# AllenInstitute/distributed-vae

Hardware: AMD Instinct MI355X
Metric: cells/sec per train step (fwd+loss+bwd+opt) (higher is better)
Workload: dtype f32; 1 GPU; cpl_mixVAE A=2 arms, synthetic-10x-v1 50000 cells x 5000 genes per GPU, batch 5000/GPU, fp32, H=100 L=10 C=92 S=2, x_drop=0.5, Adam lr=1e-3; global_batch=5000, parallelism=dp1, noise=in-kernel Philox4x32-10

## Files before the change

### distributed-vae_amd/csrc/chain.hip

```cpp
#include "common.hpp"
#include "couple.hpp"
#include <stdlib.h>
#include <type_traits>

namespace mmvae {

constexpr int CH_RT = CHAIN_ROWS / 32;
constexpr int CH_NT = 256 * CH_RT;

struct FwdLayer {
    int64_t w_off, b_off;
    int64_t out_off;
    int K, N, act;
    int64_t obn_mean_off = -1, obn_rstd_off = -1;
    int pl_slot = -1;
};
struct ChainFwdArgs {
    int nlayers;
    FwdLayer L[5];
    int64_t x_off;
    int K0;
    int64_t bn_mean_off, bn_rstd_off;
    int64_t bn_part_off;
    int part_n, part_rows;
    int64_t run_mean_off, run_var_off, run_arm_stride;
    int bn_idx;
    float bn_eps, bn_momentum;
    int64_t stats_part_off;
    int64_t acc_in_off, acc_out_off;
    int64_t planes_off;
    int planes_rows;
    int64_t wpl_off;
    int B, ld, wrows;
    int rows;
    int nblk;
    int64_t per_arm;
};

template <bool VEC>
__device__ __forceinline__ void stage_w_t(float* Ws, int ld, const float* __restrict__ W, int N, int K,
                                          int rows_pad, int cols_pad) {
    const int c4n = cols_pad >> 2;
    const int part = threadIdx.x & 7, r0 = threadIdx.x >> 3;
    for (int cb = 0; cb < c4n; cb += 32) {
        for (int row = r0; row < rows_pad; row += CH_NT / 8) {
            float4 v[4];
#pragma unroll
            for (int j = 0; j < 4; ++j) v[j] = ldg4_t<VEC>(W, K, row, (cb + part + 8 * j) * 4, N, K);
#pragma unroll
            for (int j = 0; j < 4; ++j) {
                const int c = cb + part + 8 * j;
                if (c < c4n) *reinterpret_cast<float4*>(&Ws[row * ld + c * 4]) = v[j];
            }
        }
    }
}
__device__ __forceinline__ void stage_w(float* Ws, int ld, const float* __restrict__ W, int N, int K,
                                        int rows_pad, int cols_pad) {
    const bool vec = (K & 3) == 0 && ((reinterpret_cast<uintptr_t>(W) & 15) == 0);
    if (vec) stage_w_t<true>(Ws, ld, W, N, K, rows_pad, cols_pad);
    else stage_w_t<false>(Ws, ld, W, N, K, rows_pad, cols_pad);
}

constexpr int WQ_N = 4 * (128 / (CH_NT / 8));
__device__ __forceinline__ bool w_split_ok(const float* W, int K, int rows_pad, int cols_pad) {
    return (K & 3) == 0 && ((reinterpret_cast<uintptr_t>(W) & 15) == 0) && rows_pad <= 128 && cols_pad <= 128;
}
__device__ __forceinline__ void w_load(float4 (&wq)[WQ_N], const float* __restrict__ W, int N, int K) {
    const int part = threadIdx.x & 7, r0 = threadIdx.x >> 3;
#pragma unroll
    for (int p = 0; p < WQ_N / 4; ++p)
#pragma unroll
        for (int j = 0; j < 4; ++j) {
            const int row = r0 + (CH_NT / 8) * p, col = (part + 8 * j) * 4;
            const bool ok = row < N && col < K;
            wq[p * 4 + j] = *reinterpret_cast<const float4*>(W + (int64_t)(ok ? row : 0) * K + (ok ? col : 0));
        }
}
__device__ __forceinline__ void w_store(float* Ws, int ld, const float4 (&wq)[WQ_N], int N, int K, int rows_pad, int cols_pad) {
    const int part = threadIdx.x & 7, r0 = threadIdx.x >> 3, c4n = cols_pad >> 2;
#pragma unroll
    for (int p = 0; p < WQ_N / 4; ++p)
#pragma unroll
        for (int j = 0; j < 4; ++j) {
            const int row = r0 + (CH_NT / 8) * p, c = part + 8 * j;
            const bool ok = row < N && c * 4 < K;
            const float4 q = wq[p * 4 + j];
            const float4 v = make_float4(ok ? q.x : 0.f, ok ? q.y : 0.f, ok ? q.z : 0.f, ok ? q.w : 0.f);
            if (c < c4n && row < rows_pad) *reinterpret_cast<float4*>(&Ws[row * ld + c * 4]) = v;
        }
}

typedef __bf16 bf16x8c __attribute__((ext_vector_type(8)));
typedef unsigned u32x4c __attribute__((ext_vector_type(4)));
constexpr int PLS = 128 * 128;
constexpr int WP_N = 3 * ((128 * 16) / CH_NT);
__device__ __forceinline__ void wp_load(u32x4c (&wq)[WP_N], const unsigned short* __restrict__ Wg, int N, int K) {
    const int kc_n = rup(K, 16) >> 3;
#pragma unroll
    for (int pl = 0; pl < 3; ++pl)
#pragma unroll
        for (int i = 0; i < WP_N / 3; ++i) {
            const int idx = threadIdx.x + CH_NT * i, row = idx >> 4, kc = idx & 15;
            const bool ok = row < N && kc < kc_n;
            wq[pl * (WP_N / 3) + i] = *reinterpret_cast<const u32x4c*>(Wg + pl * PLS + (ok ? row : 0) * 128 + (ok ? kc : 0) * 8);
        }
}
__device__ __forceinline__ void wp_store(unsigned* Wp, int wpl, int ldp, const u32x4c (&wq)[WP_N], int N, int K) {
    const int kc_n = rup(K, 16) >> 3;
#pragma unroll
    for (int pl = 0; pl < 3; ++pl)
#pragma unroll
        for (int i = 0; i < WP_N / 3; ++i) {
            const int idx = threadIdx.x + CH_NT * i, row = idx >> 4, kc = idx & 15;
            if (row < N && kc < kc_n) *reinterpret_cast<u32x4c*>(Wp + pl * wpl + row * ldp + kc * 4) = wq[pl * (WP_N / 3) + i];
        }
}
__device__ __forceinline__ void mma_nt_x3(f32x16& acc, const unsigned* Xp, int xpl, const unsigned* Wp, int wpl, int ldp,
                                          int a_row0, int b_row0, int ksteps) {
    const int lane = lane_id();
    const unsigned* pa = Xp + (a_row0 + (lane & 31)) * ldp + 4 * (lane >> 5);
    const unsigned* pb = Wp + (b_row0 + (lane & 31)) * ldp + 4 * (lane >> 5);
    bf16x8c a[3], b[3];
#pragma unroll
    for (int pl = 0; pl < 3; ++pl) {
        a[pl] = __builtin_bit_cast(bf16x8c, *reinterpret_cast<const u32x4c*>(pa + pl * xpl));
        b[pl] = __builtin_bit_cast(bf16x8c, *reinterpret_cast<const u32x4c*>(pb + pl * wpl));
    }
    for (int st = 0; st < ksteps; ++st) {
        const int sn = (st + 1 < ksteps) ? st + 1 : st;
        bf16x8c an[3], bn[3];
#pragma unroll
        for (int pl = 0; pl < 3; ++pl) {
            an[pl] = __builtin_bit_cast(bf16x8c, *reinterpret_cast<const u32x4c*>(pa + pl * xpl + 8 * sn));
            bn[pl] = __builtin_bit_cast(bf16x8c, *reinterpret_cast<const u32x4c*>(pb + pl * wpl + 8 * sn));
        }
        acc = __builtin_amdgcn_mfma_f32_32x32x16_bf16(a[2], b[0], acc, 0, 0, 0);
        acc = __builtin_amdgcn_mfma_f32_32x32x16_bf16(a[0], b[2], acc, 0, 0, 0);
        acc = __builtin_amdgcn_mfma_f32_32x32x16_bf16(a[1], b[1], acc, 0, 0, 0);
        acc = __builtin_amdgcn_mfma_f32_32x32x16_bf16(a[1], b[0], acc, 0, 0, 0);
        acc = __builtin_amdgcn_mfma_f32_32x32x16_bf16(a[0], b[1], acc, 0, 0, 0);
        acc = __builtin_amdgcn_mfma_f32_32x32x16_bf16(a[0], b[0], acc, 0, 0, 0);
#pragma unroll
        for (int pl = 0; pl < 3; ++pl) { a[pl] = an[pl]; b[pl] = bn[pl]; }
    }
}

template <bool X3>
__device__ __forceinline__ void chain_fwd_body(const ChainFwdArgs& a_in, const float* __restrict__ params,
                                               float* __restrict__ ws, float* __restrict__ bn_running,
                                               int64_t* __restrict__ nbt) {
    const ChainFwdArgs a = a_in;
    extern __shared__ __attribute__((aligned(16))) float smem[];
    constexpr int NPL = X3 ? 3 : 1;
    float* Xs = smem;
    float* Ws = smem + NPL * CHAIN_ROWS * a.ld;
    float* mean_s = Ws + NPL * a.wrows * a.ld;
    float* rstd_s = mean_s + 128;
    unsigned* const Xp = reinterpret_cast<unsigned*>(Xs);
    unsigned* const Wp = reinterpret_cast<unsigned*>(Ws);
    const int xpl = CHAIN_ROWS * a.ld, wpl = a.wrows * a.ld;
    const int arm = blockIdx.y, blk = blockIdx.x, b0 = blk * a.rows;
    const int tid = threadIdx.x, lane = tid & 63, wv = tid >> 6, rt = wv >> 2, ct = wv & 3;
    const int B = a.B, ld = a.ld;
    const int nvalid = min(a.rows, B - b0);
    const int Rlim = b0 + nvalid;
    const float* P = params + (int64_t)arm * a.per_arm;

    float4 wq[X3 ? 1 : WQ_N];
    u32x4c wq3[X3 ? WP_N : 1];
    bool wq_valid = false;
    const unsigned short* const WPL = reinterpret_cast<const unsigned short*>(ws + (X3 ? a.wpl_off : 0)) + (int64_t)arm * PL_SMALL_SLOTS * 3 * PLS;
    {
        const FwdLayer L0 = a.L[0];
        if constexpr (X3) {
            wq_valid = true;
            wp_load(wq3, WPL + (int64_t)L0.pl_slot * 3 * PLS, L0.N, L0.K);
        } else {
            wq_valid = w_split_ok(P + L0.w_off, L0.K, rup(L0.N, 32), rup(L0.K, 8));
            if (wq_valid) w_load(wq, P + L0.w_off, L0.N, L0.K);
        }
    }
    const float* X = ws + a.x_off + (int64_t)arm * B * a.K0;
    const int xc4n = rup(a.K0, X3 ? 16 : 8) >> 2;
    const bool x_early = (a.K0 & 3) == 0 && xc4n <= 32;
    float4 xq[4];
    if (x_early) {
#pragma unroll
        for (int j = 0; j < 4; ++j) xq[j] = ldg4_t<true>(X, a.K0, b0 + (tid >> 3), ((tid & 7) + 8 * j) * 4, Rlim, a.K0);
    }
    if (a.bn_mean_off >= 0) {
        const int K0 = a.K0;
        float mean = 0.f, rstd = 0.f;
        if (a.bn_part_off >= 0) {
            float m2 = 0.f;
            if (a.acc_in_off >= 0) {
                if (tid < K0)
                    acc_mean_m2(reinterpret_cast<const long long*>(ws + a.acc_in_off) + (int64_t)arm * ACC_SET_I64, tid, B, mean, m2);
            } else {
                stats_from_partials<CH_NT>(ws + a.bn_part_off + (int64_t)arm * a.part_n * 2 * K0, a.part_n, B, a.part_rows, K0,
                                           Ws, mean, m2);
            }
            rstd = 1.0f / sqrtf(m2 / (float)B + a.bn_eps);
            if (blk == 0 && tid < K0) {
                ws[a.bn_mean_off + (int64_t)arm * K0 + tid] = mean;
                ws[a.bn_rstd_off + (int64_t)arm * K0 + tid] = rstd;
                if (bn_running) {
                    float* rm = bn_running + a.run_mean_off + arm * a.run_arm_stride;
                    float* rv = bn_running + a.run_var_off + arm * a.run_arm_stride;
                    rm[tid] = (1.f - a.bn_momentum) * rm[tid] + a.bn_momentum * mean;
                    rv[tid] = (1.f - a.bn_momentum) * rv[tid] + a.bn_momentum * (m2 / (float)max(B - 1, 1));
                }
                if (nbt && tid == 0) nbt[arm * MMVAE_N_BN + a.bn_idx] += 1;
            }
        } else if (tid < K0) {
            mean = ws[a.bn_mean_off + (int64_t)arm * K0 + tid];
            rstd = ws[a.bn_rstd_off + (int64_t)arm * K0 + tid];
        }
        if (tid < 128) { mean_s[tid] = tid < K0 ? mean : 0.f; rstd_s[tid] = tid < K0 ? rstd : 0.f; }
        lds_barrier();
    }
    {
        const bool bn = a.bn_mean_off >= 0;
        const int c4n = xc4n;
        const bool vec = (a.K0 & 3) == 0;
        const int part = tid & 7, row = tid >> 3;
        auto stage_x = [&](auto tag) __attribute__((always_inline)) {
            constexpr bool V = decltype(tag)::value;
            for (int cb = 0; cb < c4n; cb += 32) {
                float4 v[4];
#pragma unroll
                for (int j = 0; j < 4; ++j) v[j] = (V && x_early) ? xq[j] : ldg4_t<V>(X, a.K0, b0 + row, (cb + part + 8 * j) * 4, Rlim, a.K0);
#pragma unroll
                for (int j = 0; j < 4; ++j) {
                    const int c = cb + part + 8 * j;
                    float4 o = v[j];
                    if (bn) {
                        const bool rok = b0 + row < Rlim;
                        const int cc = min(c, 31) * 4;
                        const float4 m4 = *reinterpret_cast<const float4*>(&mean_s[cc]);
                        const float4 r4 = *reinterpret_cast<const float4*>(&rstd_s[cc]);
                        o.x = rok ? (o.x - m4.x) * r4.x : 0.f;
                        o.y = rok ? (o.y - m4.y) * r4.y : 0.f;
                        o.z = rok ? (o.z - m4.z) * r4.z : 0.f;
                        o.w = rok ? (o.w - m4.w) * r4.w : 0.f;
                    }
                    if constexpr (X3) {
                        if (c < c4n) {
                            unsigned w0[3], w1[3];
                            split3(o.x, o.y, w0);
                            split3(o.z, o.w, w1);
#pragma unroll
                            for (int pl = 0; pl < 3; ++pl)
                                *reinterpret_cast<uint2*>(Xp + pl * xpl + row * ld + c * 2) = make_uint2(w0[pl], w1[pl]);
                        }
                    } else {
                        if (c < c4n) *reinterpret_cast<float4*>(&Xs[row * ld + c * 4]) = o;
                    }
                }
            }
        };
        if (vec) stage_x(VecTag{});
        else stage_x(ScalarTag{});
    }
    for (int l = 0; l < a.nlayers; ++l) {
        const FwdLayer Lr = a.L[l];
        const int K = Lr.K, N = Lr.N, KP = rup(K, 8), NPad = rup(N, 32);
        if constexpr (X3) wp_store(Wp, wpl, ld, wq3, N, K);
        else if (wq_valid) w_store(Ws, ld, wq, N, K, NPad, KP);
        else stage_w(Ws, ld, P + Lr.w_off, N, K, NPad, KP);
        const int col = ct * 32 + (lane & 31);
        const bool active = ct * 32 < NPad;
        const float bias = (active && col < N) ? P[Lr.b_off + col] : 0.f;
        const bool obn = Lr.obn_mean_off >= 0;
        const float omean = (obn && active && col < N) ? ws[Lr.obn_mean_off + (int64_t)arm * N + col] : 0.f;
        const float orstd = (obn && active && col < N) ? ws[Lr.obn_rstd_off + (int64_t)arm * N + col] : 0.f;
        lds_barrier();
        wq_valid = false;
        if (l + 1 < a.nlayers) {
            const FwdLayer Ln = a.L[l + 1];
            if constexpr (X3) {
                wp_load(wq3, WPL + (int64_t)Ln.pl_slot * 3 * PLS, Ln.N, Ln.K);
            } else {
                wq_valid = w_split_ok(P + Ln.w_off, Ln.K, rup(Ln.N, 32), rup(Ln.K, 8));
                if (wq_valid) w_load(wq, P + Ln.w_off, Ln.N, Ln.K);
            }
        }
        f32x16 acc = zero16();
        if constexpr (X3) {
            if (active) mma_nt_x3(acc, Xp, xpl, Wp, wpl, ld, rt * 32, ct * 32, rup(K, 16) >> 4);
        } else {
            if (active) mma_nt(acc, Xs, ld, rt * 32, Ws, ld, ct * 32, KP / 8);
        }
        lds_barrier();
        const bool last = (l + 1 == a.nlayers);
        const bool need_x = !last || a.planes_off >= 0;
        float vals[16];
        if (active) {
            float* out = ws + Lr.out_off + (int64_t)arm * B * N;
#pragma unroll
            for (int r = 0; r < 16; ++r) {
                const int row = rt * 32 + acc_row(r, lane);
                float v = 0.f;
                if (col < N && row < nvalid) {
                    v = acc[r] + bias;
                    if (Lr.act) v = relu_keep_nan(v);
                    out[(int64_t)(b0 + row) * N + col] = v;
                }
                vals[r] = v;
                const float xin = obn ? ((col < N && row < nvalid) ? (v - omean) * orstd : 0.f) : v;
                if constexpr (X3) {
                    const float nbv = __builtin_bit_cast(float, __builtin_amdgcn_update_dpp(0, __builtin_bit_cast(int, xin), 0xF5, 0xF, 0xF, false));
                    if (need_x && !(lane & 1) && col < rup(N, 16)) {
                        unsigned w3[3];
                        split3(xin, nbv, w3);
#pragma unroll
                        for (int pl = 0; pl < 3; ++pl) Xp[pl * xpl + row * ld + (col >> 1)] = w3[pl];
                    }
                } else {
                    if (col < rup(N, 8)) Xs[row * ld + col] = xin;
                }
            }
        }
        if (last && a.stats_part_off >= 0) {
            const int nv = max(0, min(32, nvalid - rt * 32));
            if (active) {
                float s = 0.f;
#pragma unroll
                for (int r = 0; r < 16; ++r) s += vals[r];
                s += __shfl_xor(s, 32, 64);
                const float mean = nv > 0 ? s / (float)nv : 0.f;
                float m2 = 0.f;
#pragma unroll
                for (int r = 0; r < 16; ++r) {
                    const int row = rt * 32 + acc_row(r, lane);
                    if (row < nvalid) { const float dl = vals[r] - mean; m2 += dl * dl; }
                }
                m2 += __shfl_xor(m2, 32, 64);
                if (lane < 32) { Ws[(rt * 2 + 0) * 128 + col] = mean; Ws[(rt * 2 + 1) * 128 + col] = m2; }
            }
            lds_barrier();
            if (rt == 0 && active && lane < 32 && col < N) {
                float n = 0.f, mu = 0.f, M2 = 0.f;
#pragma unroll
                for (int k = 0; k < CH_RT; ++k) {
                    const float nb = (float)max(0, min(32, nvalid - k * 32));
                    if (nb > 0.f) {
                        const float nn = n + nb, dl = Ws[(k * 2 + 0) * 128 + col] - mu;
                        mu += dl * (nb / nn);
                        M2 += Ws[(k * 2 + 1) * 128 + col] + dl * dl * (n * nb / nn);
                        n = nn;
                    }
                }
                if (a.acc_out_off >= 0) {
                    acc_add_stats(reinterpret_cast<long long*>(ws + a.acc_out_off) + (int64_t)arm * ACC_SET_I64, col, n, mu, M2);
                } else {
                    float* p = ws + a.stats_part_off + (((int64_t)arm * a.nblk + blk) * 2) * N;
                    p[col] = mu;
                    p[N + col] = M2;
                }
            }
        }
        lds_barrier();
    }
    if (a.planes_off >= 0) {
        const int N = a.L[a.nlayers - 1].N;
        const int64_t plane = (int64_t)a.planes_rows * 128;
        unsigned short* pl = reinterpret_cast<unsigned short*>(ws + a.planes_off) + (int64_t)arm * 3 * plane;
        const int rows_here = blk == a.nblk - 1 ? a.planes_rows - b0 : a.rows;
        for (int i = tid; i < rows_here * 64; i += CH_NT) {
            const int r = i >> 6, c = (i & 63) * 2;
            unsigned w[3] = {0u, 0u, 0u};
            if constexpr (X3) {
                if (r < nvalid) {
                    if (c < rup(N, 16)) {
#pragma unroll
                        for (int p = 0; p < 3; ++p) w[p] = Xp[p * xpl + r * ld + (c >> 1)];
                    }
                    if (c == N) w[0] |= 0x3F80u;
                    if (c + 1 == N) w[0] |= 0x3F800000u;
                }
            } else {
                float v0 = 0.f, v1 = 0.f;
                if (r < nvalid) {
                    v0 = c < N ? Xs[r * ld + c] : (c == N ? 1.f : 0.f);
                    v1 = c + 1 < N ? Xs[r * ld + c + 1] : (c + 1 == N ? 1.f : 0.f);
                }
                split3(v0, v1, w);
            }
#pragma unroll
            for (int p = 0; p < 3; ++p) *reinterpret_cast<unsigned*>(pl + p * plane + (int64_t)(b0 + r) * 128 + c) = w[p];
        }
    }
}
template <bool X3>
__global__ __launch_bounds__(CH_NT) void k_chain_fwd(const ChainFwdArgs a_in, const float* __restrict__ params,
                                                   float* __restrict__ ws, float* __restrict__ bn_running,
                                                   int64_t* __restrict__ nbt) {
    chain_fwd_body<X3>(a_in, params, ws, bn_running, nbt);
}

struct CoupleRoleArgs {
    int nchain, ncouple;
    int B, C;
    float eps, lam;
    int64_t cc_off, csmp_off, c_mean_off, c_iv_off, couple_part_off, c_acc_off, t_acc_off;
};
template <int AT>
__device__ __forceinline__ void couple_role(const CoupleRoleArgs& cr_in, float* __restrict__ ws) {
    const CoupleRoleArgs cr = cr_in;
    if (2 * (int)blockIdx.x >= cr.ncouple) return;
    extern __shared__ __attribute__((aligned(16))) float smem[];
    const int half = threadIdx.x >> 8, t256 = threadIdx.x & 255;
    constexpr int HALF = 4 * AT * CPL * 64 + AT * CPL * 64 + 8;
    float* sh = smem + half * HALF;
    const int blk = 2 * blockIdx.x + half;
    couple_body<AT>(blk, blk < cr.ncouple, t256, cr.B, cr.C, cr.eps, cr.lam, ws + cr.cc_off, ws + cr.csmp_off, nullptr, 0,
                    reinterpret_cast<const long long*>(ws + cr.c_acc_off), ws + cr.c_mean_off, ws + cr.c_iv_off,
                    ws + cr.couple_part_off, nullptr, reinterpret_cast<long long*>(ws + cr.t_acc_off), sh,
                    sh + 4 * AT * CPL * 64 + AT * CPL * 64, sh + 4 * AT * CPL * 64, nullptr);
}
template <int AT>
__global__ __launch_bounds__(CH_NT) void k_chain_fwd_couple(const ChainFwdArgs a_in, const CoupleRoleArgs cr_in,
                                                          const float* __restrict__ params, float* __restrict__ ws) {
    if ((int)blockIdx.y == AT) {
        couple_role<AT>(cr_in, ws);
        return;
    }
    if ((int)blockIdx.x >= cr_in.nchain) return;
    chain_fwd_body<true>(a_in, params, ws, nullptr, nullptr);
}

struct BwdLayer {
    int64_t w_off;
    int64_t dz_off;
    int64_t act_off;
    int K, N;
    int pl_slot = -1;
};
struct ChainBwdArgs {
    int nlayers;
    BwdLayer L[5];
    int64_t g_off;
    int nslab;
    int64_t slab_stride;
    int64_t bnb_part_off;
    int bnb_n;
    int64_t bn_mean_off, bn_rstd_off;
    int64_t gout_off;
    int64_t part_off;
    int64_t rprev_off, rprev_mean_off, rprev_rstd_off;
    int64_t acc_in_off, acc_out_off, zero_off;
    int zero_n4;
    int64_t wpl_off;
    int B, ld, wrows;
    int64_t per_arm;
};

__device__ __forceinline__ float bn_bwd_val(float g, float av, float mm, float rr, float s1, float s2, float invB) {
#pragma clang fp contract(off)
    const float xh = (av - mm) * rr;
    const float t = g - s1 * invB;
    const float u = xh * (s2 * invB);
    return rr * (t - u);
}
__device__ __forceinline__ float bn_bwd_xhat_acc(float g, float rprev, float mu, float rs, float sum) {
#pragma clang fp contract(off)
    const float xh = (rprev - mu) * rs;
    const float p = g * xh;
    return sum + p;
}

template <bool X3>
__global__ __launch_bounds__(CH_NT) void k_chain_bwd(const ChainBwdArgs a_in, const float* __restrict__ params,
                                                   float* __restrict__ ws) {
    const ChainBwdArgs a = a_in;
    extern __shared__ __attribute__((aligned(16))) float smem[];
    constexpr int NPL = X3 ? 3 : 1;
    float* Gs = smem;
    float* Ws = smem + NPL * CHAIN_ROWS * a.ld;
    float* sums_s = Ws + NPL * a.wrows * a.ld;
    unsigned* const Gp = reinterpret_cast<unsigned*>(Gs);
    unsigned* const Wp = reinterpret_cast<unsigned*>(Ws);
    const int xpl = CHAIN_ROWS * a.ld, wpl = a.wrows * a.ld;
    const int arm = blockIdx.y, blk = blockIdx.x, b0 = blk * CHAIN_ROWS;
    const int tid = threadIdx.x, lane = tid & 63, wv = tid >> 6, rt = wv >> 2, ct = wv & 3;
    const int B = a.B, ld = a.ld;
    const int nvalid = min(CHAIN_ROWS, B - b0);
    const float* P = params + (int64_t)arm * a.per_arm;

    if (a.zero_n4 > 0) grid_zero(ws + a.zero_off, a.zero_n4);
    if (a.bnb_part_off >= 0 && a.acc_in_off >= 0) {
        const int N = a.L[0].N;
        if (tid < 128) {
            double s1 = 0.0, s2 = 0.0;
            if (tid < N) acc_get(reinterpret_cast<const long long*>(ws + a.acc_in_off) + (int64_t)arm * ACC_SET_I64, tid, s1, s2);
            sums_s[tid] = (float)s1;
            sums_s[128 + tid] = (float)s2;
        }
        lds_barrier();
    } else if (a.bnb_part_off >= 0) {
        const int N = a.L[0].N;
        const float r = sums_from_partials<CH_NT>(ws + a.bnb_part_off + (int64_t)arm * a.bnb_n * 2 * N, a.bnb_n, 2 * N,
                                                  reinterpret_cast<double*>(Ws));
        if (tid < 256) sums_s[tid] = 0.f;
        lds_barrier();
        if (tid < 2 * N) sums_s[tid < N ? tid : 128 + tid - N] = r;
        lds_barrier();
    }
    {
        const BwdLayer L0 = a.L[0];
        const int N = L0.N, c4n = rup(N, X3 ? 16 : 8) >> 2;
        const bool has_act = L0.act_off >= 0, bnb = a.bnb_part_off >= 0;
        const float* G = ws + a.g_off + (int64_t)arm * B * N;
        const float* act = has_act ? ws + L0.act_off + (int64_t)arm * B * N : G;
        float* dz = ws + L0.dz_off + (int64_t)arm * B * N;
        const float* mu = bnb ? ws + a.bn_mean_off + (int64_t)arm * N : G;
        const float* rs = bnb ? ws + a.bn_rstd_off + (int64_t)arm * N : G;
        const float invB = 1.f / (float)B;
        const bool vec = (N & 3) == 0;
        const int part = tid & 7, row = tid >> 3;
        const bool rok = row < nvalid;
        auto stage_g = [&](auto tag) __attribute__((always_inline)) {
            constexpr bool V = decltype(tag)::value;
            for (int cb = 0; cb < c4n; cb += 32) {
                float4 gq[4], avq[4], mmq[4], rrq[4];
#pragma unroll
                for (int j = 0; j < 4; ++j) {
                    const int col = (cb + part + 8 * j) * 4;
                    float4 g = make_float4(0.f, 0.f, 0.f, 0.f);
                    auto add_slabs = [&](auto chunk) __attribute__((always_inline)) {
                        constexpr int CHK = decltype(chunk)::value;
                        for (int s0 = 0; s0 < a.nslab; s0 += CHK) {
                            float4 t[CHK];
#pragma unroll
                            for (int sl = 0; sl < CHK; ++sl)
                                t[sl] = ldg4_t<V>(G + (int64_t)min(s0 + sl, a.nslab - 1) * a.slab_stride, N, b0 + row, col, B, N);
#pragma unroll
                            for (int sl = 0; sl < CHK; ++sl) {
                                const bool on = s0 + sl < a.nslab;
                                g.x += on ? t[sl].x : 0.f; g.y += on ? t[sl].y : 0.f; g.z += on ? t[sl].z : 0.f; g.w += on ? t[sl].w : 0.f;
                            }
                        }
                    };
                    if (a.nslab == 1) g = ldg4_t<V>(G, N, b0 + row, col, B, N);
                    else if (a.nslab <= 4) add_slabs(std::integral_constant<int, 4>{});
                    else add_slabs(std::integral_constant<int, 16>{});
                    gq[j] = g;
                    avq[j] = ldg4_t<V>(act, N, b0 + row, col, B, N);
                    mmq[j] = ldg4_t<V>(mu, 0, 0, col, 1, N);
                    rrq[j] = ldg4_t<V>(rs, 0, 0, col, 1, N);
                }
#pragma unroll
                for (int j = 0; j < 4; ++j) {
                    const int c = cb + part + 8 * j, col = c * 4;
                    float4 g = gq[j];
                    const float4 av = avq[j];
                    if (bnb) {
                        const int cs = min(c, 31) * 4;
                        const float4 m1 = *reinterpret_cast<const float4*>(&sums_s[cs]);
                        const float4 m2 = *reinterpret_cast<const float4*>(&sums_s[128 + cs]);
                        const float4 mm = mmq[j], rr = rrq[j];
                        g.x = bn_bwd_val(g.x, av.x, mm.x, rr.x, m1.x, m2.x, invB);
                        g.y = bn_bwd_val(g.y, av.y, mm.y, rr.y, m1.y, m2.y, invB);
                        g.z = bn_bwd_val(g.z, av.z, mm.z, rr.z, m1.z, m2.z, invB);
                        g.w = bn_bwd_val(g.w, av.w, mm.w, rr.w, m1.w, m2.w, invB);
                    }
                    float4 v;
                    v.x = (rok && col < N && (!has_act || av.x > 0.f)) ? g.x : 0.f;
                    v.y = (rok && col + 1 < N && (!has_act || av.y > 0.f)) ? g.y : 0.f;
                    v.z = (rok && col + 2 < N && (!has_act || av.z > 0.f)) ? g.z : 0.f;
                    v.w = (rok && col + 3 < N && (!has_act || av.w > 0.f)) ? g.w : 0.f;
                    if (c < c4n) {
                        if constexpr (X3) {
                            unsigned w0[3], w1[3];
                            split3(v.x, v.y, w0);
                            split3(v.z, v.w, w1);
#pragma unroll
                            for (int pl = 0; pl < 3; ++pl)
                                *reinterpret_cast<uint2*>(Gp + pl * xpl + row * ld + c * 2) = make_uint2(w0[pl], w1[pl]);
                        } else {
                            *reinterpret_cast<float4*>(&Gs[row * ld + col]) = v;
                        }
                        if (rok) {
                            float* o = dz + (int64_t)(b0 + row) * N + col;
                            if (V && col + 3 < N) *reinterpret_cast<float4*>(o) = v;
                            else {
                                if (col < N) o[0] = v.x;
                                if (col + 1 < N) o[1] = v.y;
                                if (col + 2 < N) o[2] = v.z;
                                if (col + 3 < N) o[3] = v.w;
                            }
                        }
                    }
                }
            }
        };
        if (vec) stage_g(VecTag{});
        else stage_g(ScalarTag{});
    }
    float4 wq[X3 ? 1 : WQ_N];
    u32x4c wq3[X3 ? WP_N : 1];
    bool wq_valid = false;
    const unsigned short* const WPL = reinterpret_cast<const unsigned short*>(ws + (X3 ? a.wpl_off : 0)) + (int64_t)arm * PL_SMALL_SLOTS * 3 * PLS;
    if constexpr (X3) wp_load(wq3, WPL + (int64_t)a.L[0].pl_slot * 3 * PLS, a.L[0].K, a.L[0].N);
    for (int l = 0; l < a.nlayers; ++l) {
        const BwdLayer Lr = a.L[l];
        const int K = Lr.K, N = Lr.N, NP8 = rup(N, 8), KPad = rup(K, 32);
        if constexpr (X3) wp_store(Wp, wpl, ld, wq3, K, N);
        else if (wq_valid) w_store(Ws, ld, wq, N, K, NP8, KPad);
        else stage_w(Ws, ld, P + Lr.w_off, N, K, NP8, KPad);
        lds_barrier();
        wq_valid = false;
        if (l + 1 < a.nlayers) {
            const BwdLayer Ln = a.L[l + 1];
            if constexpr (X3) {
                wp_load(wq3, WPL + (int64_t)Ln.pl_slot * 3 * PLS, Ln.K, Ln.N);
            } else {
                wq_valid = w_split_ok(P + Ln.w_off, Ln.K, rup(Ln.N, 8), rup(Ln.K, 32));
                if (wq_valid) w_load(wq, P + Ln.w_off, Ln.N, Ln.K);
            }
        }
        const bool last = (l + 1 == a.nlayers);
        constexpr int NTI = X3 ? 1 : 2;
        float pre[NTI][16];
        {
            const float* src = nullptr;
            if (!last) {
                const BwdLayer Ln = a.L[l + 1];
                src = Ln.act_off >= 0 ? ws + Ln.act_off + (int64_t)arm * B * K : nullptr;
            } else if (a.part_off >= 0) {
                src = ws + a.rprev_off + (int64_t)arm * B * K;
            }
#pragma unroll
            for (int ti = 0; ti < NTI; ++ti) {
                const int col = (ct + 4 * ti) * 32 + (lane & 31);
#pragma unroll
                for (int r = 0; r < 16; ++r) {
                    const int row = rt * 32 + acc_row(r, lane);
                    const bool ok = src && (ct + 4 * ti) * 32 < KPad && col < K && row < nvalid;
                    pre[ti][r] = ok ? src[(int64_t)(b0 + row) * K + col] : (last ? 0.f : 1.f);
                }
            }
        }
        f32x16 accs[NTI];
#pragma unroll
        for (int ti = 0; ti < NTI; ++ti) accs[ti] = zero16();
#pragma unroll
        for (int ti = 0; ti < NTI; ++ti) {
            const int cti = ct + 4 * ti;
            if constexpr (X3) {
                if (cti * 32 < KPad) mma_nt_x3(accs[ti], Gp, xpl, Wp, wpl, ld, rt * 32, cti * 32, rup(N, 16) >> 4);
            } else {
                if (cti * 32 < KPad) mma_nn(accs[ti], Gs, ld, rt * 32, Ws, ld, cti * 32, NP8 / 8);
            }
        }
        lds_barrier();
        float ps1[2] = {0.f, 0.f}, ps2[2] = {0.f, 0.f};
#pragma unroll
        for (int ti = 0; ti < NTI; ++ti) {
            const int cti = ct + 4 * ti;
            if (cti * 32 >= KPad) continue;
            const f32x16 acc = accs[ti];
            const int col = cti * 32 + (lane & 31);
            if (!last) {
                const BwdLayer Ln = a.L[l + 1];
                float* dz = ws + Ln.dz_off + (int64_t)arm * B * K;
#pragma unroll
                for (int r = 0; r < 16; ++r) {
                    const int row = rt * 32 + acc_row(r, lane);
                    const bool ok = col < K && row < nvalid;
                    const float v = (ok && pre[ti][r] > 0.f) ? acc[r] : 0.f;
                    if (ok) dz[(int64_t)(b0 + row) * K + col] = v;
                    if constexpr (X3) {
                        const float nbv = __builtin_bit_cast(float, __builtin_amdgcn_update_dpp(0, __builtin_bit_cast(int, v), 0xF5, 0xF, 0xF, false));
                        if (!(lane & 1) && col < rup(K, 16)) {
                            unsigned w3[3];
                            split3(v, nbv, w3);
#pragma unroll
                            for (int pl = 0; pl < 3; ++pl) Gp[pl * xpl + row * ld + (col >> 1)] = w3[pl];
                        }
                    } else {
                        Gs[row * ld + col] = v;
                    }
                }
            } else {
                float* go = ws + a.gout_off + (int64_t)arm * B * K;
                float s1 = 0.f, s2 = 0.f;
                const bool want = a.part_off >= 0;
                float mu = 0.f, rs = 0.f;
                if (want && col < K) {
                    mu = ws[a.rprev_mean_off + (int64_t)arm * K + col];
                    rs = ws[a.rprev_rstd_off + (int64_t)arm * K + col];
                }
#pragma unroll
                for (int r = 0; r < 16; ++r) {
                    const int row = rt * 32 + acc_row(r, lane);
                    if (col < K && row < nvalid) {
                        go[(int64_t)(b0 + row) * K + col] = acc[r];
                        s1 += acc[r];
                        s2 = bn_bwd_xhat_acc(acc[r], pre[ti][r], mu, rs, s2);
                    }
                }
                if (want) {
                    s1 += __shfl_xor(s1, 32, 64);
                    s2 += __shfl_xor(s2, 32, 64);
                    ps1[ti] = s1;
                    ps2[ti] = s2;
                }
            }
        }
        if (last && a.part_off >= 0) {
#pragma unroll
            for (int ti = 0; ti < NTI; ++ti) {
                const int col = (ct + 4 * ti) * 32 + (lane & 31);
                if (lane < 32) { Ws[(rt * 2 + 0) * 256 + col] = ps1[ti]; Ws[(rt * 2 + 1) * 256 + col] = ps2[ti]; }
            }
            lds_barrier();
            if (tid < K) {
                float t1 = 0.f, t2 = 0.f;
#pragma unroll
                for (int k = 0; k < CH_RT; ++k) { t1 += Ws[(k * 2 + 0) * 256 + tid]; t2 += Ws[(k * 2 + 1) * 256 + tid]; }
                if (a.acc_out_off >= 0) {
                    acc_add_sums(reinterpret_cast<long long*>(ws + a.acc_out_off) + (int64_t)arm * ACC_SET_I64, tid, t1, t2);
                } else {
                    float* p = ws + a.part_off + (((int64_t)arm * gridDim.x + blk) * 2) * K;
                    p[tid] = t1;
                    p[K + tid] = t2;
                }
            }
        }
        lds_barrier();
    }
}

__global__ __launch_bounds__(256) void k_bn_bwd_apply(const float* __restrict__ G, const float* __restrict__ R,
                                                      const float* __restrict__ mean, const float* __restrict__ rstd,
                                                      const float* __restrict__ part, int npart,
                                                      const long long* __restrict__ acc, float* __restrict__ DZ,
                                                      int B, int W, unsigned short* __restrict__ planes, int Rp) {
    __shared__ __attribute__((aligned(16))) double scratch[1024];
    __shared__ float sums_s[2][128], mu_s[128], rs_s[128];
    const int arm = blockIdx.y, blk = blockIdx.x, tid = threadIdx.x;
    if (acc) {
        if (tid < W) {
            double s1, s2;
            acc_get(acc + (int64_t)arm * ACC_SET_I64, tid, s1, s2);
            sums_s[0][tid] = (float)s1;
            sums_s[1][tid] = (float)s2;
        }
    } else {
        const float r = sums_from_partials<256>(part + (int64_t)arm * npart * 2 * W, npart, 2 * W, scratch);
        if (tid < 2 * W) sums_s[tid < W ? 0 : 1][tid < W ? tid : tid - W] = r;
    }
    if (tid < W) { mu_s[tid] = mean[arm * W + tid]; rs_s[tid] = rstd[arm * W + tid]; }
    lds_barrier();
    const float invB = 1.f / (float)B;
    const int nvalid = max(0, min(32, B - blk * 32));
    const int64_t base = ((int64_t)arm * B + (int64_t)blk * 32) * W;
    auto dz_of = [&](float gv, float rv, int col) {
        const float rs = rs_s[col];
        const float xh = (rv - mu_s[col]) * rs;
        const float g = rs * (gv - sums_s[0][col] * invB - xh * (sums_s[1][col] * invB));
        return rv > 0.f ? g : 0.f;
    };
    if (!planes) {
        for (int i = tid; i < nvalid * W; i += 256) DZ[base + i] = dz_of(G[base + i], R[base + i], i % W);
        return;
    }
    const int64_t plane = (int64_t)Rp * 128;
    unsigned short* pl = planes + (int64_t)arm * 3 * plane;
#pragma unroll
    for (int it = 0; it < 8; ++it) {
        const int i = tid + 256 * it, r = i >> 6, c = (i & 63) * 2, row = blk * 32 + r;
        const bool ok = r < nvalid && c < W;
        const int64_t o = base + (int64_t)(ok ? r : 0) * W + (ok ? c : 0);
        float2 d = make_float2(0.f, 0.f);
        if (nvalid > 0) {
            const float2 gv = *reinterpret_cast<const float2*>(G + o), rv = *reinterpret_cast<const float2*>(R + o);
            if (ok) {
                d = make_float2(dz_of(gv.x, rv.x, c), dz_of(gv.y, rv.y, c + 1));
                *reinterpret_cast<float2*>(DZ + o) = d;
            }
        }
        if (row < Rp) {
            unsigned w[3];
            split3(d.x, d.y, w);
#pragma unroll
            for (int p = 0; p < 3; ++p) *reinterpret_cast<unsigned*>(pl + p * plane + (int64_t)row * 128 + c) = w[p];
        }
    }
}

constexpr int WS_SCRATCH = 8192;
static int fwd_ld(int maxdim) { return rup(maxdim, 8) + 4; }
static int bwd_ld(int maxdim) { return rup(maxdim, 32) + 4; }
static size_t chain_smem(int ld, int wrows) { return (size_t)(CHAIN_ROWS * ld + wrows * ld + 256) * sizeof(float); }
static int x3_ld(int maxdim) { return rup(maxdim, 16) / 2 + 4; }
static size_t chain_smem_x3(int ld, int wrows) { return (size_t)(3 * CHAIN_ROWS * ld + 3 * wrows * ld + 256) * sizeof(float); }
static int launch_fwd(const Ctx& c, ChainFwdArgs& a, int maxdim, const float* params, float* bn_running, int64_t* nbt, const char* what) {
    a.rows = c.lay.chain_rows_fwd;
    a.nblk = c.lay.nblkf;
    const dim3 grid(c.lay.nblkf, c.d.A);
    if (c.plan.chain_planes) {
        a.ld = x3_ld(maxdim);
        a.wrows = 128;
        a.wpl_off = c.lay.pl_small;
        const size_t shm = chain_smem_x3(a.ld, a.wrows);
        hipLaunchKernelGGL(k_chain_fwd<true>, grid, dim3(CH_NT), shm, c.stream, a, params, c.ws, bn_running, nbt);
    } else {
        hipLaunchKernelGGL(k_chain_fwd<false>, grid, dim3(CH_NT), chain_smem(a.ld, a.wrows), c.stream, a, params, c.ws, bn_running, nbt);
    }
    HIP_LAUNCH_CHECK(what);
    return 0;
}

static int launch_bwd(const Ctx& c, ChainBwdArgs& a, int maxdim, const float* params, const char* what) {
    const dim3 grid(c.lay.nblkc, c.d.A);
    if (c.plan.chain_planes) {
        a.ld = x3_ld(maxdim);
        a.wrows = 128;
        a.wpl_off = c.lay.pl_small;
        const size_t shm = chain_smem_x3(a.ld, a.wrows);
        hipLaunchKernelGGL(k_chain_bwd<true>, grid, dim3(CH_NT), shm, c.stream, a, params, c.ws);
    } else {
        hipLaunchKernelGGL(k_chain_bwd<false>, grid, dim3(CH_NT), chain_smem(a.ld, a.wrows), c.stream, a, params, c.ws);
    }
    HIP_LAUNCH_CHECK(what);
    return 0;
}

int launch_chain_fwd_enc(const Ctx& c, int layer, const float* params, float* bn_running, int64_t* nbt) {
    const mmvae_dims& d = c.d;
    const Layout& L = c.lay;
    ChainFwdArgs a{};
    a.nlayers = 1;
    const int i = layer - 1;
    const int N = (layer == 5) ? d.L : d.H;
    a.L[0] = FwdLayer{c.po.o[2 * (layer - 1)], c.po.o[2 * (layer - 1) + 1], L.R[i], d.H, N, 1};
    a.x_off = L.R[i - 1];
    a.K0 = d.H;
    a.bn_mean_off = L.bn_mean[i - 1];
    a.bn_rstd_off = L.bn_rstd[i - 1];
    a.bn_part_off = c.h.training ? L.bn_part[i - 1] : -1;
    a.part_n = (layer == 2) ? L.nblk32 : L.nblkf;
    a.part_rows = (layer == 2) ? 32 : L.chain_rows_fwd;
    a.run_mean_off = c.po.bn_mean[i - 1];
    a.run_var_off = c.po.bn_var[i - 1];
    a.run_arm_stride = c.po.bn_per_arm;
    a.bn_idx = i - 1;
    a.bn_eps = c.h.eps;
    a.bn_momentum = c.h.bn_momentum;
// ... 166 lines not shown
```

Baseline: 7.647 million cells/s.

## Use AMD buffer resource loads/stores with OOB clamping in chain fwd/bwd kernels

Replaces per-element bounds-checked global loads and stores in the chain forward/backward kernels with raw buffer loads/stores on per-block buffer resource descriptors. Out-of-range lanes get an offset past the buffer size, so hardware bounds checking returns zero or drops the store instead of relying on branches and 64-bit address math. The change also unrolls the split-bf16 MFMA k-loop by two with double-buffered fragments. It relies on OOB loads returning zero, which changes some default fill values (for example the ungated pre path now uses a gated flag) and on 32-bit byte offsets fitting within a block.

New measurement: 7.779 million cells/s (median of 6 runs). +1.7%, better.

```diff
diff --git a/distributed-vae_amd/csrc/chain.hip b/distributed-vae_amd/csrc/chain.hip
--- a/distributed-vae_amd/csrc/chain.hip
+++ b/distributed-vae_amd/csrc/chain.hip
@@ -37,6 +37,45 @@
     int64_t per_arm;
 };
 
+typedef __bf16 bf16x8c __attribute__((ext_vector_type(8)));
+typedef unsigned u32x4c __attribute__((ext_vector_type(4)));
+constexpr uint32_t CH_BLOCK_BYTES = (uint32_t)CHAIN_ROWS * 256u * 4u, CH_OOB = 0x80000000u;
+static_assert(CH_BLOCK_BYTES < CH_OOB && (uint64_t)CH_BLOCK_BYTES + CH_OOB <= 0xFFFFFFFFull,
+              "32-bit byte offsets within a workgroup's rows");
+__device__ __forceinline__ __amdgpu_buffer_rsrc_t ch_rsrc(const float* p, int rows, int width) {
+    return __builtin_amdgcn_make_buffer_rsrc(const_cast<float*>(p), 0, max(rows, 0) * width * 4, 0x00020000);
+}
+__device__ __forceinline__ float ch_ld(__amdgpu_buffer_rsrc_t rs, uint32_t byte_off) {
+    return __builtin_bit_cast(float, (uint32_t)__builtin_amdgcn_raw_buffer_load_b32(rs, (int)byte_off, 0, 0));
+}
+__device__ __forceinline__ void ch_st(__amdgpu_buffer_rsrc_t rs, uint32_t byte_off, float v) {
+    __builtin_amdgcn_raw_buffer_store_b32(__builtin_bit_cast(uint32_t, v), rs, (int)byte_off, 0, 0);
+}
+template <bool VEC>
+__device__ __forceinline__ float4 ch_ld4(__amdgpu_buffer_rsrc_t rs, uint32_t row_off, int col, int Cn) {
+    const uint32_t o = row_off + (uint32_t)col * 4u;
+    if (VEC) return __builtin_bit_cast(float4, __builtin_amdgcn_raw_buffer_load_b128(rs, (int)(col < Cn ? o : CH_OOB), 0, 0));
+    float4 v;
+    v.x = ch_ld(rs, col < Cn ? o : CH_OOB);
+    v.y = ch_ld(rs, col + 1 < Cn ? o + 4u : CH_OOB);
+    v.z = ch_ld(rs, col + 2 < Cn ? o + 8u : CH_OOB);
+    v.w = ch_ld(rs, col + 3 < Cn ? o + 12u : CH_OOB);
+    return v;
+}
+
+template <bool VEC>
+__device__ __forceinline__ void ch_st4(__amdgpu_buffer_rsrc_t rs, uint32_t row_off, int col, int Cn, float4 v) {
+    const uint32_t o = row_off + (uint32_t)col * 4u;
+    if (VEC) {
+        __builtin_amdgcn_raw_buffer_store_b128(__builtin_bit_cast(u32x4c, v), rs, (int)(col < Cn ? o : CH_OOB), 0, 0);
+        return;
+    }
+    ch_st(rs, col < Cn ? o : CH_OOB, v.x);
+    ch_st(rs, col + 1 < Cn ? o + 4u : CH_OOB, v.y);
+    ch_st(rs, col + 2 < Cn ? o + 8u : CH_OOB, v.z);
+    ch_st(rs, col + 3 < Cn ? o + 12u : CH_OOB, v.w);
+}
+
 template <bool VEC>
 __device__ __forceinline__ void stage_w_t(float* Ws, int ld, const float* __restrict__ W, int N, int K,
                                           int rows_pad, int cols_pad) {
@@ -68,14 +107,12 @@
 }
 __device__ __forceinline__ void w_load(float4 (&wq)[WQ_N], const float* __restrict__ W, int N, int K) {
     const int part = threadIdx.x & 7, r0 = threadIdx.x >> 3;
+    const auto rW = ch_rsrc(W, N, K);
 #pragma unroll
     for (int p = 0; p < WQ_N / 4; ++p)
 #pragma unroll
-        for (int j = 0; j < 4; ++j) {
-            const int row = r0 + (CH_NT / 8) * p, col = (part + 8 * j) * 4;
-            const bool ok = row < N && col < K;
-            wq[p * 4 + j] = *reinterpret_cast<const float4*>(W + (int64_t)(ok ? row : 0) * K + (ok ? col : 0));
-        }
+        for (int j = 0; j < 4; ++j)
+            wq[p * 4 + j] = ch_ld4<true>(rW, (uint32_t)((r0 + (CH_NT / 8) * p) * K) * 4u, (part + 8 * j) * 4, K);
 }
 __device__ __forceinline__ void w_store(float* Ws, int ld, const float4 (&wq)[WQ_N], int N, int K, int rows_pad, int cols_pad) {
     const int part = threadIdx.x & 7, r0 = threadIdx.x >> 3, c4n = cols_pad >> 2;
@@ -84,27 +121,23 @@
 #pragma unroll
         for (int j = 0; j < 4; ++j) {
             const int row = r0 + (CH_NT / 8) * p, c = part + 8 * j;
-            const bool ok = row < N && c * 4 < K;
-            const float4 q = wq[p * 4 + j];
-            const float4 v = make_float4(ok ? q.x : 0.f, ok ? q.y : 0.f, ok ? q.z : 0.f, ok ? q.w : 0.f);
-            if (c < c4n && row < rows_pad) *reinterpret_cast<float4*>(&Ws[row * ld + c * 4]) = v;
-        }
-}
-
-typedef __bf16 bf16x8c __attribute__((ext_vector_type(8)));
-typedef unsigned u32x4c __attribute__((ext_vector_type(4)));
+            if (c < c4n && row < rows_pad) *reinterpret_cast<float4*>(&Ws[row * ld + c * 4]) = wq[p * 4 + j];
+        }
+}
+
 constexpr int PLS = 128 * 128;
 constexpr int WP_N = 3 * ((128 * 16) / CH_NT);
 __device__ __forceinline__ void wp_load(u32x4c (&wq)[WP_N], const unsigned short* __restrict__ Wg, int N, int K) {
+    const auto rW = __builtin_amdgcn_make_buffer_rsrc(const_cast<unsigned short*>(Wg), 0, 3 * PLS * 2, 0x00020000);
     const int kc_n = rup(K, 16) >> 3;
 #pragma unroll
-    for (int pl = 0; pl < 3; ++pl)
-#pragma unroll
-        for (int i = 0; i < WP_N / 3; ++i) {
-            const int idx = threadIdx.x + CH_NT * i, row = idx >> 4, kc = idx & 15;
-            const bool ok = row < N && kc < kc_n;
-            wq[pl * (WP_N / 3) + i] = *reinterpret_cast<const u32x4c*>(Wg + pl * PLS + (ok ? row : 0) * 128 + (ok ? kc : 0) * 8);
-        }
+    for (int i = 0; i < WP_N / 3; ++i) {
+        const int idx = threadIdx.x + CH_NT * i, row = idx >> 4, kc = idx & 15;
+        const uint32_t off = (row < N && kc < kc_n) ? threadIdx.x * 16u : CH_OOB;
+#pragma unroll
+        for (int pl = 0; pl < 3; ++pl)
+            wq[pl * (WP_N / 3) + i] = __builtin_bit_cast(u32x4c, __builtin_amdgcn_raw_buffer_load_b128(rW, (int)off, (pl * PLS + CH_NT * i * 8) * 2, 0));
+    }
 }
 __device__ __forceinline__ void wp_store(unsigned* Wp, int wpl, int ldp, const u32x4c (&wq)[WP_N], int N, int K) {
     const int kc_n = rup(K, 16) >> 3;
@@ -115,35 +148,38 @@
             const int idx = threadIdx.x + CH_NT * i, row = idx >> 4, kc = idx & 15;
             if (row < N && kc < kc_n) *reinterpret_cast<u32x4c*>(Wp + pl * wpl + row * ldp + kc * 4) = wq[pl * (WP_N / 3) + i];
         }
+}
+struct FragX3 { bf16x8c a[3], b[3]; };
+__device__ __forceinline__ void frag_x3(FragX3& f, const unsigned* pa, int xpl, const unsigned* pb, int wpl, int st) {
+#pragma unroll
+    for (int pl = 0; pl < 3; ++pl) {
+        f.a[pl] = __builtin_bit_cast(bf16x8c, *reinterpret_cast<const u32x4c*>(pa + pl * xpl + 8 * st));
+        f.b[pl] = __builtin_bit_cast(bf16x8c, *reinterpret_cast<const u32x4c*>(pb + pl * wpl + 8 * st));
+    }
+}
+__device__ __forceinline__ void mfma6_x3(f32x16& acc, const FragX3& f) {
+    acc = __builtin_amdgcn_mfma_f32_32x32x16_bf16(f.a[2], f.b[0], acc, 0, 0, 0);
+    acc = __builtin_amdgcn_mfma_f32_32x32x16_bf16(f.a[0], f.b[2], acc, 0, 0, 0);
+    acc = __builtin_amdgcn_mfma_f32_32x32x16_bf16(f.a[1], f.b[1], acc, 0, 0, 0);
+    acc = __builtin_amdgcn_mfma_f32_32x32x16_bf16(f.a[1], f.b[0], acc, 0, 0, 0);
+    acc = __builtin_amdgcn_mfma_f32_32x32x16_bf16(f.a[0], f.b[1], acc, 0, 0, 0);
+    acc = __builtin_amdgcn_mfma_f32_32x32x16_bf16(f.a[0], f.b[0], acc, 0, 0, 0);
 }
 __device__ __forceinline__ void mma_nt_x3(f32x16& acc, const unsigned* Xp, int xpl, const unsigned* Wp, int wpl, int ldp,
                                           int a_row0, int b_row0, int ksteps) {
     const int lane = lane_id();
     const unsigned* pa = Xp + (a_row0 + (lane & 31)) * ldp + 4 * (lane >> 5);
     const unsigned* pb = Wp + (b_row0 + (lane & 31)) * ldp + 4 * (lane >> 5);
-    bf16x8c a[3], b[3];
-#pragma unroll
-    for (int pl = 0; pl < 3; ++pl) {
-        a[pl] = __builtin_bit_cast(bf16x8c, *reinterpret_cast<const u32x4c*>(pa + pl * xpl));
-        b[pl] = __builtin_bit_cast(bf16x8c, *reinterpret_cast<const u32x4c*>(pb + pl * wpl));
-    }
-    for (int st = 0; st < ksteps; ++st) {
-        const int sn = (st + 1 < ksteps) ? st + 1 : st;
-        bf16x8c an[3], bn[3];
-#pragma unroll
-        for (int pl = 0; pl < 3; ++pl) {
-            an[pl] = __builtin_bit_cast(bf16x8c, *reinterpret_cast<const u32x4c*>(pa + pl * xpl + 8 * sn));
-            bn[pl] = __builtin_bit_cast(bf16x8c, *reinterpret_cast<const u32x4c*>(pb + pl * wpl + 8 * sn));
-        }
-        acc = __builtin_amdgcn_mfma_f32_32x32x16_bf16(a[2], b[0], acc, 0, 0, 0);
-        acc = __builtin_amdgcn_mfma_f32_32x32x16_bf16(a[0], b[2], acc, 0, 0, 0);
-        acc = __builtin_amdgcn_mfma_f32_32x32x16_bf16(a[1], b[1], acc, 0, 0, 0);
-        acc = __builtin_amdgcn_mfma_f32_32x32x16_bf16(a[1], b[0], acc, 0, 0, 0);
-        acc = __builtin_amdgcn_mfma_f32_32x32x16_bf16(a[0], b[1], acc, 0, 0, 0);
-        acc = __builtin_amdgcn_mfma_f32_32x32x16_bf16(a[0], b[0], acc, 0, 0, 0);
-#pragma unroll
-        for (int pl = 0; pl < 3; ++pl) { a[pl] = an[pl]; b[pl] = bn[pl]; }
-    }
+    FragX3 f0, f1;
+    frag_x3(f0, pa, xpl, pb, wpl, 0);
+    int st = 0;
+    for (; st + 1 < ksteps; st += 2) {
+        frag_x3(f1, pa, xpl, pb, wpl, st + 1);
+        mfma6_x3(acc, f0);
+        frag_x3(f0, pa, xpl, pb, wpl, min(st + 2, ksteps - 1));
+        mfma6_x3(acc, f1);
+    }
+    if (st < ksteps) mfma6_x3(acc, f0);
 }
 
 template <bool X3>
@@ -165,6 +201,7 @@
     const int B = a.B, ld = a.ld;
     const int nvalid = min(a.rows, B - b0);
     const int Rlim = b0 + nvalid;
+    const uint32_t row_l = (uint32_t)(rt * 32 + 4 * (lane >> 5));
     const float* P = params + (int64_t)arm * a.per_arm;
 
     float4 wq[X3 ? 1 : WQ_N];
@@ -181,13 +218,14 @@
             if (wq_valid) w_load(wq, P + L0.w_off, L0.N, L0.K);
         }
     }
-    const float* X = ws + a.x_off + (int64_t)arm * B * a.K0;
+    const auto rX = ch_rsrc(ws + a.x_off + ((int64_t)arm * B + b0) * a.K0, nvalid, a.K0);
+    const uint32_t x_row = (uint32_t)((tid >> 3) * a.K0) * 4u;
     const int xc4n = rup(a.K0, X3 ? 16 : 8) >> 2;
     const bool x_early = (a.K0 & 3) == 0 && xc4n <= 32;
     float4 xq[4];
     if (x_early) {
 #pragma unroll
-        for (int j = 0; j < 4; ++j) xq[j] = ldg4_t<true>(X, a.K0, b0 + (tid >> 3), ((tid & 7) + 8 * j) * 4, Rlim, a.K0);
+        for (int j = 0; j < 4; ++j) xq[j] = ch_ld4<true>(rX, x_row, ((tid & 7) + 8 * j) * 4, a.K0);
     }
     if (a.bn_mean_off >= 0) {
         const int K0 = a.K0;
@@ -230,7 +268,7 @@
             for (int cb = 0; cb < c4n; cb += 32) {
                 float4 v[4];
 #pragma unroll
-                for (int j = 0; j < 4; ++j) v[j] = (V && x_early) ? xq[j] : ldg4_t<V>(X, a.K0, b0 + row, (cb + part + 8 * j) * 4, Rlim, a.K0);
+                for (int j = 0; j < 4; ++j) v[j] = (V && x_early) ? xq[j] : ch_ld4<V>(rX, x_row, (cb + part + 8 * j) * 4, a.K0);
 #pragma unroll
                 for (int j = 0; j < 4; ++j) {
                     const int c = cb + part + 8 * j;
@@ -271,10 +309,11 @@
         else stage_w(Ws, ld, P + Lr.w_off, N, K, NPad, KP);
         const int col = ct * 32 + (lane & 31);
         const bool active = ct * 32 < NPad;
-        const float bias = (active && col < N) ? P[Lr.b_off + col] : 0.f;
+        const uint32_t c_off = (active && col < N) ? (uint32_t)col * 4u : CH_OOB;
+        const float bias = ch_ld(ch_rsrc(P + Lr.b_off, 1, N), c_off);
         const bool obn = Lr.obn_mean_off >= 0;
-        const float omean = (obn && active && col < N) ? ws[Lr.obn_mean_off + (int64_t)arm * N + col] : 0.f;
-        const float orstd = (obn && active && col < N) ? ws[Lr.obn_rstd_off + (int64_t)arm * N + col] : 0.f;
+        const float omean = ch_ld(ch_rsrc(ws + Lr.obn_mean_off + (int64_t)arm * N, obn ? 1 : 0, N), c_off);
+        const float orstd = ch_ld(ch_rsrc(ws + Lr.obn_rstd_off + (int64_t)arm * N, obn ? 1 : 0, N), c_off);
         lds_barrier();
         wq_valid = false;
         if (l + 1 < a.nlayers) {
@@ -297,16 +336,15 @@
         const bool need_x = !last || a.planes_off >= 0;
         float vals[16];
         if (active) {
-            float* out = ws + Lr.out_off + (int64_t)arm * B * N;
+            const auto rO = ch_rsrc(ws + Lr.out_off + ((int64_t)arm * B + b0) * N, nvalid, N);
+            const uint32_t o_lane = col < N ? (row_l * (uint32_t)N + (uint32_t)col) * 4u : CH_OOB;
 #pragma unroll
             for (int r = 0; r < 16; ++r) {
                 const int row = rt * 32 + acc_row(r, lane);
-                float v = 0.f;
-                if (col < N && row < nvalid) {
-                    v = acc[r] + bias;
-                    if (Lr.act) v = relu_keep_nan(v);
-                    out[(int64_t)(b0 + row) * N + col] = v;
-                }
+                float v = acc[r] + bias;
+                if (Lr.act) v = relu_keep_nan(v);
+                v = (col < N && row < nvalid) ? v : 0.f;
+                ch_st(rO, o_lane + (uint32_t)(acc_row(r, 0) * N) * 4u, v);
                 vals[r] = v;
                 const float xin = obn ? ((col < N && row < nvalid) ? (v - omean) * orstd : 0.f) : v;
                 if constexpr (X3) {
@@ -366,7 +404,7 @@
     if (a.planes_off >= 0) {
         const int N = a.L[a.nlayers - 1].N;
         const int64_t plane = (int64_t)a.planes_rows * 128;
-        unsigned short* pl = reinterpret_cast<unsigned short*>(ws + a.planes_off) + (int64_t)arm * 3 * plane;
+        char* const pl = reinterpret_cast<char*>(reinterpret_cast<unsigned short*>(ws + a.planes_off) + (int64_t)arm * 3 * plane + (int64_t)b0 * 128);
         const int rows_here = blk == a.nblk - 1 ? a.planes_rows - b0 : a.rows;
         for (int i = tid; i < rows_here * 64; i += CH_NT) {
             const int r = i >> 6, c = (i & 63) * 2;
@@ -389,7 +427,7 @@
                 split3(v0, v1, w);
             }
 #pragma unroll
-            for (int p = 0; p < 3; ++p) *reinterpret_cast<unsigned*>(pl + p * plane + (int64_t)(b0 + r) * 128 + c) = w[p];
+            for (int p = 0; p < 3; ++p) *reinterpret_cast<unsigned*>(pl + p * plane * 2 + (uint32_t)(r * 128 + c) * 2u) = w[p];
         }
     }
 }
@@ -487,6 +525,7 @@
     const int tid = threadIdx.x, lane = tid & 63, wv = tid >> 6, rt = wv >> 2, ct = wv & 3;
     const int B = a.B, ld = a.ld;
     const int nvalid = min(CHAIN_ROWS, B - b0);
+    const uint32_t row_l = (uint32_t)(rt * 32 + 4 * (lane >> 5));
     const float* P = params + (int64_t)arm * a.per_arm;
 
     if (a.zero_n4 > 0) grid_zero(ws + a.zero_off, a.zero_n4);
@@ -512,15 +551,18 @@
         const BwdLayer L0 = a.L[0];
         const int N = L0.N, c4n = rup(N, X3 ? 16 : 8) >> 2;
         const bool has_act = L0.act_off >= 0, bnb = a.bnb_part_off >= 0;
-        const float* G = ws + a.g_off + (int64_t)arm * B * N;
-        const float* act = has_act ? ws + L0.act_off + (int64_t)arm * B * N : G;
-        float* dz = ws + L0.dz_off + (int64_t)arm * B * N;
-        const float* mu = bnb ? ws + a.bn_mean_off + (int64_t)arm * N : G;
-        const float* rs = bnb ? ws + a.bn_rstd_off + (int64_t)arm * N : G;
+        const int64_t blk_off = ((int64_t)arm * B + b0) * N;
+        const float* G = ws + a.g_off + blk_off;
+        const auto rG = ch_rsrc(G, nvalid, N);
+        const auto rAct = has_act ? ch_rsrc(ws + L0.act_off + blk_off, nvalid, N) : rG;
+        const auto rDz = ch_rsrc(ws + L0.dz_off + blk_off, nvalid, N);
+        const auto rMu = ch_rsrc(ws + a.bn_mean_off + (int64_t)arm * N, bnb ? 1 : 0, N);
+        const auto rRs = ch_rsrc(ws + a.bn_rstd_off + (int64_t)arm * N, bnb ? 1 : 0, N);
         const float invB = 1.f / (float)B;
         const bool vec = (N & 3) == 0;
         const int part = tid & 7, row = tid >> 3;
         const bool rok = row < nvalid;
+        const uint32_t g_row = (uint32_t)(row * N) * 4u;
         auto stage_g = [&](auto tag) __attribute__((always_inline)) {
             constexpr bool V = decltype(tag)::value;
             for (int cb = 0; cb < c4n; cb += 32) {
@@ -535,21 +577,19 @@
                             float4 t[CHK];
 #pragma unroll
                             for (int sl = 0; sl < CHK; ++sl)
-                                t[sl] = ldg4_t<V>(G + (int64_t)min(s0 + sl, a.nslab - 1) * a.slab_stride, N, b0 + row, col, B, N);
-#pragma unroll
-                            for (int sl = 0; sl < CHK; ++sl) {
-                                const bool on = s0 + sl < a.nslab;
-                                g.x += on ? t[sl].x : 0.f; g.y += on ? t[sl].y : 0.f; g.z += on ? t[sl].z : 0.f; g.w += on ? t[sl].w : 0.f;
-                            }
+                                t[sl] = ch_ld4<V>(ch_rsrc(G + (int64_t)min(s0 + sl, a.nslab - 1) * a.slab_stride,
+                                                          s0 + sl < a.nslab ? nvalid : 0, N), g_row, col, N);
+#pragma unroll
+                            for (int sl = 0; sl < CHK; ++sl) { g.x += t[sl].x; g.y += t[sl].y; g.z += t[sl].z; g.w += t[sl].w; }
                         }
                     };
-                    if (a.nslab == 1) g = ldg4_t<V>(G, N, b0 + row, col, B, N);
+                    if (a.nslab == 1) g = ch_ld4<V>(rG, g_row, col, N);
                     else if (a.nslab <= 4) add_slabs(std::integral_constant<int, 4>{});
                     else add_slabs(std::integral_constant<int, 16>{});
                     gq[j] = g;
-                    avq[j] = ldg4_t<V>(act, N, b0 + row, col, B, N);
-                    mmq[j] = ldg4_t<V>(mu, 0, 0, col, 1, N);
-                    rrq[j] = ldg4_t<V>(rs, 0, 0, col, 1, N);
+                    avq[j] = ch_ld4<V>(rAct, g_row, col, N);
+                    mmq[j] = ch_ld4<V>(rMu, 0u, col, N);
+                    rrq[j] = ch_ld4<V>(rRs, 0u, col, N);
                 }
 #pragma unroll
                 for (int j = 0; j < 4; ++j) {
@@ -582,17 +622,8 @@
                         } else {
                             *reinterpret_cast<float4*>(&Gs[row * ld + col]) = v;
                         }
-                        if (rok) {
-                            float* o = dz + (int64_t)(b0 + row) * N + col;
-                            if (V && col + 3 < N) *reinterpret_cast<float4*>(o) = v;
-                            else {
-                                if (col < N) o[0] = v.x;
-                                if (col + 1 < N) o[1] = v.y;
-                                if (col + 2 < N) o[2] = v.z;
-                                if (col + 3 < N) o[3] = v.w;
-                            }
-                        }
                     }
+                    ch_st4<V>(rDz, g_row, col, N, v);
                 }
             }
         };
@@ -624,23 +655,19 @@
         const bool last = (l + 1 == a.nlayers);
         constexpr int NTI = X3 ? 1 : 2;
         float pre[NTI][16];
+        const int64_t blk_off = ((int64_t)arm * B + b0) * K;
+        const int64_t pre_off = last ? a.rprev_off : a.L[last ? l : l + 1].act_off;
+        const bool gated = !last && pre_off >= 0;
+        uint32_t o_lane[NTI];
         {
-            const float* src = nullptr;
-            if (!last) {
-                const BwdLayer Ln = a.L[l + 1];
-                src = Ln.act_off >= 0 ? ws + Ln.act_off + (int64_t)arm * B * K : nullptr;
-            } else if (a.part_off >= 0) {
-                src = ws + a.rprev_off + (int64_t)arm * B * K;
-            }
+            const bool has_src = last ? a.part_off >= 0 : pre_off >= 0;
+            const auto rPre = ch_rsrc(ws + pre_off + blk_off, has_src ? nvalid : 0, K);
 #pragma unroll
             for (int ti = 0; ti < NTI; ++ti) {
                 const int col = (ct + 4 * ti) * 32 + (lane & 31);
-#pragma unroll
-                for (int r = 0; r < 16; ++r) {
-                    const int row = rt * 32 + acc_row(r, lane);
-                    const bool ok = src && (ct + 4 * ti) * 32 < KPad && col < K && row < nvalid;
-                    pre[ti][r] = ok ? src[(int64_t)(b0 + row) * K + col] : (last ? 0.f : 1.f);
-                }
+                o_lane[ti] = ((ct + 4 * ti) * 32 < KPad && col < K) ? (row_l * (uint32_t)K + (uint32_t)col) * 4u : CH_OOB;
+#pragma unroll
+                for (int r = 0; r < 16; ++r) pre[ti][r] = ch_ld(rPre, o_lane[ti] + (uint32_t)(acc_row(r, 0) * K) * 4u);
             }
         }
         f32x16 accs[NTI];
@@ -664,14 +691,13 @@
             const f32x16 acc = accs[ti];
             const int col = cti * 32 + (lane & 31);
             if (!last) {
-                const BwdLayer Ln = a.L[l + 1];
-                float* dz = ws + Ln.dz_off + (int64_t)arm * B * K;
+                const auto rDz = ch_rsrc(ws + a.L[l + 1].dz_off + blk_off, nvalid, K);
 #pragma unroll
                 for (int r = 0; r < 16; ++r) {
                     const int row = rt * 32 + acc_row(r, lane);
                     const bool ok = col < K && row < nvalid;
-                    const float v = (ok && pre[ti][r] > 0.f) ? acc[r] : 0.f;
-                    if (ok) dz[(int64_t)(b0 + row) * K + col] = v;
+                    const float v = (ok && (!gated || pre[ti][r] > 0.f)) ? acc[r] : 0.f;
+                    ch_st(rDz, o_lane[ti] + (uint32_t)(acc_row(r, 0) * K) * 4u, v);
                     if constexpr (X3) {
                         const float nbv = __builtin_bit_cast(float, __builtin_amdgcn_update_dpp(0, __builtin_bit_cast(int, v), 0xF5, 0xF, 0xF, false));
                         if (!(lane & 1) && col < rup(K, 16)) {
@@ -685,19 +711,17 @@
                     }
                 }
             } else {
-                float* go = ws + a.gout_off + (int64_t)arm * B * K;
+                const auto rGo = ch_rsrc(ws + a.gout_off + blk_off, nvalid, K);
                 float s1 = 0.f, s2 = 0.f;
                 const bool want = a.part_off >= 0;
-                float mu = 0.f, rs = 0.f;
-                if (want && col < K) {
-                    mu = ws[a.rprev_mean_off + (int64_t)arm * K + col];
-                    rs = ws[a.rprev_rstd_off + (int64_t)arm * K + col];
-                }
+                const uint32_t c_off = col < K ? (uint32_t)col * 4u : CH_OOB;
+                const float mu = ch_ld(ch_rsrc(ws + a.rprev_mean_off + (int64_t)arm * K, want ? 1 : 0, K), c_off);
+                const float rs = ch_ld(ch_rsrc(ws + a.rprev_rstd_off + (int64_t)arm * K, want ? 1 : 0, K), c_off);
 #pragma unroll
                 for (int r = 0; r < 16; ++r) {
                     const int row = rt * 32 + acc_row(r, lane);
+                    ch_st(rGo, o_lane[ti] + (uint32_t)(acc_row(r, 0) * K) * 4u, acc[r]);
                     if (col < K && row < nvalid) {
-                        go[(int64_t)(b0 + row) * K + col] = acc[r];
                         s1 += acc[r];
                         s2 = bn_bwd_xhat_acc(acc[r], pre[ti][r], mu, rs, s2);
                     }
```
